# Epiphany-f/PSL-SLAM

Hardware: AMD Instinct MI355X
Metric: frames/sec ORB+line extract+match, 640x480 RGB-D, 1/2/4/8 MI355X (higher is better)
Workload: dtype u8; 1 GPU; configs[2]: 640x480 synthetic structure scene at the configured line load ('sticks': non-overlapping high-contrast bars), ORB 1000/1.2/8 FAST 20/7 + LSD (LSD_REFINE_ADV) / merge / top-200 / LBD + LIL pairing + RGB-D line glue (isLineGood, crossings, planes) extract, SearchByProjection(cur,last) + LSDmatcher::match, frames resident in HBM; scene=sticks, distinct_frames_per_batch=256, streams=1, launcher=none, multi_gpu=single GPU, lsd_refine=LSD_REFINE_ADV, lbd_sample_bytes_per_frame=2654242

## Files before the change

### psl-slam_amd/csrc/pslfe_line.hip

```cpp
#include <math.h>
#include <stdlib.h>
#include <string.h>

#include <algorithm>
#include <mutex>
#include <vector>

#include "line_kernels2.h"
#include "line_kernels3.h"
#include "pslfe_internal.h"

#ifndef PSL_NFA_COUNT_WGS
#define PSL_NFA_COUNT_WGS 4
#endif
#define PSL_GROW_LDS_USED_MAX (144u * 1024u)
#ifndef PSL_GROW_HELPER_FRAMES
#define PSL_GROW_HELPER_FRAMES 64
#endif

#define PSL_GROW_LDS_DEVICES 64
static std::mutex g_grow_lds_mu;
static size_t g_grow_lds_attr[PSL_GROW_LDS_DEVICES];

static hipError_t psl_grow_lds_allow(int device, size_t bytes) {
    if (bytes <= 64u * 1024u) return hipSuccess;
    if (device < 0 || device >= PSL_GROW_LDS_DEVICES) return hipErrorInvalidDevice;
    std::lock_guard<std::mutex> lock(g_grow_lds_mu);
    if (bytes <= g_grow_lds_attr[device]) return hipSuccess;
    const hipError_t e = hipFuncSetAttribute(reinterpret_cast<const void*>(&k_lsd_grow4<3, 1>), hipFuncAttributeMaxDynamicSharedMemorySize, (int)bytes);
    if (e == hipSuccess) g_grow_lds_attr[device] = bytes;
    return e;
}

struct pslfe_line {
    pslfe_ctx* ctx = nullptr;
    int numOctaves = 1, nfeatures = 200, max_batch = 1;
    float scale = 1.2f;
    double min_line_length = 0;
    int refine = 2;
    std::vector<float> scaleF, invScaleF, sigma2, invSigma2;

    int gw = 0, gh = 0;
    LineParams P;
    size_t in_fstride = 0;
    int in_pitch = 0;
    int last_nframes = 0;

    uint8_t* d_in = nullptr;
    double* d_scaled = nullptr;
    float* d_angdeg = nullptr;
    double* d_modgrad = nullptr;
    float2* d_trig = nullptr;
    float2* d_seedt = nullptr;
    uint8_t* d_used = nullptr;
    uint32_t* d_reg = nullptr;
    LsdnTables NT = {};
    double* d_lgamma = nullptr;
    double* d_sctab = nullptr;
    double* d_rects = nullptr;
    int* d_nrect = nullptr;
    int* d_weight = nullptr;
    int* d_order = nullptr;
    float* d_segtmp = nullptr;
    uint8_t* d_keep = nullptr;
    int2* d_counts = nullptr;
    int2* d_count0 = nullptr;
    uint16_t* d_ulist = nullptr;
    int* d_ucount = nullptr;
    double* d_vals = nullptr;
    double2* d_sstate = nullptr;
    LsdnSeries* d_slist = nullptr;
    LsdnSeries* d_stmp = nullptr;
    int* d_lcount = nullptr;
    float* d_seg = nullptr;
    int* d_nseg = nullptr;
    MergeScratch M = {};
    PslKeyLine* d_kls = nullptr;
    uint8_t* d_ldesc = nullptr;
    float* d_fdesc = nullptr;
    double* d_lineEq = nullptr;
    int* d_nkl = nullptr;
    int* d_status = nullptr;
    short2* d_dxy = nullptr;
    float* d_rawfans = nullptr;
    float* d_fans = nullptr;
    int* d_nfans = nullptr;
    float* d_tmplines = nullptr;

    PslDeviceBuffers mem;

    void release() {
        mem.release();
        gw = gh = 0;
        last_nframes = 0;
    }

    int prepare(int w, int h) {
        if (w == gw && h == gh) return PSLFE_OK;
        PSL_REQUIRE(w >= 16 && h >= 16 && w <= 8192 && h <= 8192, PSLFE_E_INVALID, "line: image %dx%d out of range", w, h);
        LineParams Q;
        memset(&Q, 0, sizeof(Q));
        Q.w = w; Q.h = h;
        Q.W = (int)nearbyint(w * 0.8);
        Q.H = (int)nearbyint(h * 0.8);
        Q.maxseg = PSL_MERGE_NMAX;
        Q.maxkl = std::max(1024, nfeatures);
        Q.nfeatures = nfeatures;
        {
            const double sigma = 0.6 / 0.8;
            const int ksize = 1 + 2 * (int)ceil(sigma * sqrt(2 * 3.0 * log(10.0)));
            PSL_REQUIRE(ksize == 7, PSLFE_E_INVALID, "line: unexpected LSD kernel size %d", ksize);
            const double scale2X = -0.5 / (sigma * sigma);
            double sum = 0;
            for (int i = 0; i < 7; ++i) { const double x = i - 3.0; Q.gk[i] = exp(scale2X * x * x); sum += Q.gk[i]; }
            sum = 1. / sum;
            for (int i = 0; i < 7; ++i) Q.gk[i] *= sum;
        }
        Q.prec = PSL_PI * 22.5 / 180;
        Q.p = 22.5 / 180;
        Q.rho = 2.0 / sin(Q.prec);
        {
            double q = Q.rho * Q.rho;
            while (sqrt(nextafter(q, INFINITY)) <= Q.rho) q = nextafter(q, INFINITY);
            while (sqrt(q) > Q.rho) q = nextafter(q, 0.0);
            Q.rho_q = q;
        }
        const double LOG_NT = 5 * (log10((double)Q.W) + log10((double)Q.H)) / 2 + log10(11.0);
        Q.min_reg_size = (int)(size_t)(-LOG_NT / log10(Q.p));
        Q.log_nt = LOG_NT;
        Q.refine = refine;
        {
            float cf[5];
            double sum = 0;
            for (int i = 0; i < 5; ++i) { const double x = i - 2.0; cf[i] = (float)exp(-0.5 * x * x); sum += cf[i]; }
            sum = 1. / sum;
            for (int i = 0; i < 5; ++i) { cf[i] = (float)(cf[i] * sum); Q.lbdK[i] = (int)nearbyint((double)cf[i] * 256.0); }
        }
        {
            const int wb = 7, nb = 9;
            double u = (wb * 3 - 1) / 2, sigma = (wb * 2 + 1) / 2, inv = -1 / (2 * sigma * sigma);
            for (int i = 0; i < wb * 3; ++i) { const double d = i - u; Q.gaussL[i] = (float)exp(d * d * inv); }
            u = (nb * wb - 1) / 2; sigma = u; inv = -1 / (2 * sigma * sigma);
            for (int i = 0; i < nb * wb; ++i) { const double d = i - u; Q.gaussG[i] = (float)exp(d * d * inv); }
        }
        PSL_HIP(hipSetDevice(ctx->device));
        PSL_HIP(hipStreamSynchronize(ctx->stream));
        release();
        if (int rc = allocate(Q, w, h)) { release(); return rc; }
        P = Q;
        gw = w; gh = h;
        last_nframes = 0;
        return PSLFE_OK;
    }

    int allocate(LineParams& Q, int w, int h) {
        const size_t F = (size_t)max_batch, npx = (size_t)Q.W * Q.H, N = PSL_MERGE_NMAX;
        in_pitch = (int)psl_align_up(w, 16);
        in_fstride = psl_align_up((size_t)in_pitch * h, 256);
        static const double sctab[444] = {
#include "psl_sincostab.inc"
        };
        const int lgn = 1 << 16;
        std::vector<double> lg((size_t)lgn, 0.0);
        for (int i = 1; i < lgn; ++i) lg[i] = lsdn_log_gamma((double)i);
        lg.resize((size_t)lgn + 3 * PSL_NFA_NP + PSL_RATIO_BMAX);
        for (int i = 1; i < PSL_RATIO_BMAX; ++i) lg[(size_t)lgn + 3 * PSL_NFA_NP + i] = 1.0 / (double)i;
        double pj = Q.p;
        for (int j = 0; j < PSL_NFA_NP; ++j, pj = pj / 2) {
            lg[(size_t)lgn + j] = psl_log(pj); lg[(size_t)lgn + PSL_NFA_NP + j] = psl_log(1.0 - pj); lg[(size_t)lgn + 2 * PSL_NFA_NP + j] = psl_log10(pj);
        }
        mem.alloc(d_in, in_fstride * F, "d_in");
        mem.alloc(d_scaled, npx * std::min<size_t>(F, PSL_LSD_SUBBATCH), "d_scaled");
        mem.alloc(d_angdeg, npx * F, "d_angdeg");
        mem.alloc(d_modgrad, npx * F, "d_modgrad");
        mem.alloc(d_trig, npx * F, "d_trig");
        mem.alloc(d_seedt, npx * F, "d_seedt");
        mem.alloc(d_used, npx * F, "d_used");
        mem.alloc(d_reg, npx * F, "d_reg");
        mem.alloc(d_seg, (size_t)Q.maxseg * 4 * F, "d_seg");
        mem.alloc(d_nseg, F, "d_nseg");
        mem.alloc(d_rects, (size_t)Q.maxseg * PSL_LSD_RECT_F64 * F, "d_rects");
        mem.alloc(d_nrect, F, "d_nrect");
        mem.alloc(d_weight, F, "d_weight");
        mem.alloc(d_order, F, "d_order");
        mem.alloc(d_segtmp, (size_t)Q.maxseg * 4 * F, "d_segtmp");
        mem.alloc(d_keep, (size_t)Q.maxseg * F, "d_keep");
        mem.alloc(d_counts, (size_t)Q.maxseg * 5 * F, "d_counts");
        mem.alloc(d_count0, (size_t)Q.maxseg * F, "d_count0");
        mem.alloc(d_ulist, (size_t)Q.maxseg * 2 * F, "d_ulist");
        mem.alloc(d_ucount, 5 * F, "d_ucount");
        mem.alloc(d_vals, (size_t)Q.maxseg * 5 * F, "d_vals");
        mem.alloc(d_sstate, (size_t)Q.maxseg * 5 * F, "d_sstate");
        mem.alloc(d_slist, (size_t)Q.maxseg * 5 * F, "d_slist");
        mem.alloc(d_stmp, (size_t)Q.maxseg * 5 * F, "d_stmp");
        mem.alloc(d_lcount, F * (PSL_NFA_NCLS + 1), "d_lcount");
        mem.alloc(d_sctab, sizeof(sctab) / sizeof(double), "d_sctab");
        mem.alloc(d_lgamma, lg.size(), "d_lgamma");
        mem.alloc(M.lines0, F * N * 4, "M.lines0");
        mem.alloc(M.lines1, F * N * 4, "M.lines1");
        mem.alloc(M.merged, F * N * 4, "M.merged");
        mem.alloc(M.angles, F * N, "M.angles");
        mem.alloc(M.length, F * N, "M.length");
        mem.alloc(M.order, F * N, "M.order");
        mem.alloc(M.pos, F * N, "M.pos");
        mem.alloc(M.adj, F * N * (N / 32), "M.adj");
        mem.alloc(M.code, F * N, "M.code");
        mem.alloc(M.clist, F * PSL_MERGE_CLMAX, "M.clist");
        mem.alloc(M.coff, F * (2 * N + 2), "M.coff");
        mem.alloc(M.work, F * 4 * N, "M.work");
        mem.alloc(M.bits, F * (N / 32), "M.bits");
        mem.alloc(M.stage, F * N, "M.stage");
        mem.alloc(d_kls, F * Q.maxkl, "d_kls");
        mem.alloc(d_ldesc, F * Q.maxkl * 32, "d_ldesc");
        mem.alloc(d_fdesc, F * Q.maxkl * 72, "d_fdesc");
        mem.alloc(d_lineEq, F * Q.maxkl * 3, "d_lineEq");
        mem.alloc(d_nkl, F, "d_nkl");
        mem.alloc(d_status, F, "d_status");
        mem.alloc(d_dxy, F * (size_t)w * h, "d_dxy");
        mem.alloc(d_rawfans, F * PSL_FAN_CAP * 4, "d_rawfans");
        mem.alloc(d_fans, F * PSL_FAN_CAP * 4, "d_fans");
        mem.alloc(d_nfans, F, "d_nfans");
        mem.alloc(d_tmplines, N * 4, "d_tmplines");
        if (int rc = mem.check("line")) return rc;
        PSL_HIP(hipMemcpy(d_sctab, sctab, sizeof(sctab), hipMemcpyHostToDevice));
        Q.sctab = d_sctab;
        PSL_HIP(hipMemcpy(d_lgamma, lg.data(), lg.size() * sizeof(double), hipMemcpyHostToDevice));
        NT.lg = d_lgamma; NT.logs = d_lgamma + lgn; NT.lg_n = lgn; NT.p0 = Q.p; NT.log_nt = Q.log_nt; NT.inv = d_lgamma + lgn + 3 * PSL_NFA_NP;
        return PSLFE_OK;
    }

    int run_lsd(const uint8_t* d_gray, int nframes, int w, int h, int stride, size_t frame_stride) {
        int rc = prepare(w, h);
        if (rc) return rc;
        PSL_HIP(hipSetDevice(ctx->device));
        hipStream_t st = ctx->stream;
        const unsigned F = (unsigned)nframes;
        {
            PSL_HIP(hipMemsetAsync(d_used, 0, (size_t)P.W * P.H * F, st));
            P.singles = F <= PSL_GROW_HELPER_FRAMES;
            P.full_grad = nframes == 1;
            const bool ordered = F > PSL_GROW_HELPER_FRAMES;
            if (ordered) PSL_HIP(hipMemsetAsync(d_weight, 0, (size_t)F * sizeof(int), st));
            const unsigned tx = (P.W + 63) / 64, ty = (P.H + 15) / 16, gy = (P.H + PSL_GRAD_TH - 1) / PSL_GRAD_TH;
            const size_t npx = (size_t)P.W * P.H;
            for (unsigned f0 = 0; f0 < F; f0 += PSL_LSD_SUBBATCH) {
                const unsigned n = std::min<unsigned>(PSL_LSD_SUBBATCH, F - f0);
                const int xcd = n >= 8 ? 1 : 0;
                const size_t po = (size_t)f0 * npx;
                {
                    PSL_STAGE_BEGIN(ctx, "line.lsd_scale");
                    k_lsd_scale_tiled<<<xcd ? dim3(8, tx * ty, (n + 7) / 8) : dim3(tx, ty, n), 256, 0, st>>>(P, d_gray + (size_t)f0 * frame_stride, stride, frame_stride,
                                                                                                             d_scaled, (int)n, xcd);
                    PSL_STAGE_END(ctx, "line.lsd_scale");
                }
                {
                    PSL_STAGE_BEGIN(ctx, "line.lsd_grad");
                    k_lsd_grad<<<xcd ? dim3(8, tx * gy, (n + 7) / 8) : dim3(tx, gy, n), 256, 0, st>>>(P, d_scaled, d_angdeg + po, d_modgrad + po, d_trig + po, d_seedt + po,
                                                                                                      d_used + po, ordered ? d_weight + f0 : nullptr, (int)n, xcd);
                    PSL_STAGE_END(ctx, "line.lsd_grad");
                }
            }
            if (ordered) k_frame_order<<<1, 1024, 0, st>>>(d_weight, (int)F, P.W * P.H, d_order);
        }
        P.refine = refine;
        {
            PSL_STAGE_BEGIN(ctx, "line.lsd_grow");
            if (F <= PSL_GROW_HELPER_FRAMES) {
                const size_t ubytes = (((size_t)P.W * P.H + 31) >> 5) * 4;
                if (ubytes <= PSL_GROW_LDS_USED_MAX) {
                    PSL_HIP(psl_grow_lds_allow(ctx->device, ubytes));
                    k_lsd_grow4<3, 1><<<F, 256, ubytes, st>>>(P, d_angdeg, d_modgrad, d_trig, d_used, d_seedt, d_reg, d_seg, refine >= 2 ? d_nrect : d_nseg, d_rects, (int)F, nullptr);
                } else {
                    k_lsd_grow4<3, 0><<<F, 256, 0, st>>>(P, d_angdeg, d_modgrad, d_trig, d_used, d_seedt, d_reg, d_seg, refine >= 2 ? d_nrect : d_nseg, d_rects, (int)F, nullptr);
                }
            } else
                k_lsd_grow4<0, 0><<<F, 64, 0, st>>>(P, d_angdeg, d_modgrad, d_trig, d_used, d_seedt, d_reg, d_seg, refine >= 2 ? d_nrect : d_nseg, d_rects, (int)F,
                                                 d_order);
            PSL_STAGE_END(ctx, "line.lsd_grow");
            PSL_HIP(hipGetLastError());
        }
        if (refine >= 2) {
            const dim3 gc(F >= 64 ? PSL_NFA_COUNT_WGS : 128, F), gs(F >= 64 ? 1 : 4, F);
            PSL_HIP(hipMemsetAsync(d_ucount, 0, (size_t)5 * F * sizeof(int), st));
            auto ul = [&](int k) { return k >= 0 ? d_ulist + (size_t)(k & 1) * P.maxseg * F : nullptr; };
            auto uc = [&](int k) { return k >= 0 && k < 5 ? d_ucount + (size_t)k * F : nullptr; };
#define PSL_NFA_COUNT(PH)                                                                                                \
    {                                                                                                                    \
        PSL_STAGE_BEGIN(ctx, "line.nfa_count");                                                                          \
        k_lsd_nfa_count<PH><<<gc, 256, 0, st>>>(P, d_angdeg, d_rects, d_nrect, ul(PH + 1), uc(PH + 1), d_counts, d_count0); \
        PSL_STAGE_END(ctx, "line.nfa_count");                                                                            \
    }
#define PSL_NFA_EVAL(PH)                                                                                                 \
    {                                                                                                                    \
        PSL_STAGE_BEGIN(ctx, "line.nfa_eval");                                                                           \
        k_lsd_nfa_setup<PH><<<F, 256, 0, st>>>(P, NT, d_rects, d_nrect, ul(PH + 1), uc(PH + 1), d_counts, d_count0, d_vals, d_sstate, d_stmp, d_slist, d_lcount); \
        k_lsd_nfa_series<PH><<<dim3(PSL_NFA_NCLS, (F + PSL_NFA_FG - 1) / PSL_NFA_FG), 256, 0, st>>>(P, NT, (int)F, d_slist, d_lcount, d_sstate); \
        k_lsd_nfa_select<PH><<<gs, 256, 0, st>>>(P, NT.log_nt, d_rects, d_nrect, ul(PH + 1), uc(PH + 1), d_keep, d_vals, d_sstate, d_segtmp, \
                                                 PH < 3 ? ul(PH + 2) : nullptr, uc(PH + 2));                             \
        PSL_STAGE_END(ctx, "line.nfa_eval");                                                                             \
    }
            PSL_NFA_COUNT(PSL_NFA_FIRST)
            PSL_NFA_EVAL(PSL_NFA_FIRST)
            PSL_NFA_EVAL(-1)
            PSL_NFA_COUNT(0)
            PSL_NFA_EVAL(0)
            PSL_NFA_COUNT(1)
            PSL_NFA_EVAL(1)
            PSL_NFA_COUNT(2)
            PSL_NFA_EVAL(2)
            PSL_NFA_COUNT(3)
            PSL_NFA_EVAL(3)
#undef PSL_NFA_COUNT
#undef PSL_NFA_EVAL
            k_lsd_emit<<<F, 256, 0, st>>>(P, d_nrect, d_segtmp, d_keep, d_seg, d_nseg);
        }
        PSL_HIP(hipGetLastError());
        last_nframes = nframes;
        return PSLFE_OK;
    }

    int run_merge(int nframes) {
        PSL_HIP(hipSetDevice(ctx->device));
        PSL_STAGE_BEGIN(ctx, "line.merge");
        k_line_merge<PSL_MERGE_LDSN_SMALL><<<nframes, 256, 0, ctx->stream>>>(P, M, d_seg, d_nseg, d_kls, d_lineEq, d_nkl, d_status);
        k_line_merge<PSL_MERGE_LDSN><<<nframes, 256, 0, ctx->stream>>>(P, M, d_seg, d_nseg, d_kls, d_lineEq, d_nkl, d_status);
        PSL_STAGE_END(ctx, "line.merge");
        PSL_HIP(hipGetLastError());
        return PSLFE_OK;
    }

    int run_lbd(const uint8_t* d_gray, int nframes, int stride, size_t frame_stride, bool want_float) {
        PSL_HIP(hipSetDevice(ctx->device));
        hipStream_t st = ctx->stream;
        {
            PSL_STAGE_BEGIN(ctx, "line.lbd_pre");
            const unsigned tx = (P.w + 63) / 64, ty = (P.h + 31) / 32;
            const int xcd = nframes >= 8 ? 1 : 0;
            k_lbd_pre<<<xcd ? dim3(8, tx * ty, (nframes + 7) / 8) : dim3(tx, ty, nframes), 256, 0, st>>>(P, d_gray, stride, frame_stride, d_dxy, nframes, xcd);
            PSL_STAGE_END(ctx, "line.lbd_pre");
        }
        {
            PSL_STAGE_BEGIN(ctx, "line.lbd");
            const int per_frame = std::min(P.maxkl, std::max(P.nfeatures, 1));
            k_lbd<<<dim3((per_frame + 3) / 4, nframes), 256, 0, st>>>(P, d_dxy, d_kls, d_nkl, d_ldesc, want_float ? d_fdesc : nullptr);
            PSL_STAGE_END(ctx, "line.lbd");
        }
        PSL_HIP(hipGetLastError());
        return PSLFE_OK;
    }

    int run_pair(int nframes, float radius, float fanThr) {
        PSL_HIP(hipSetDevice(ctx->device));
        PSL_STAGE_BEGIN(ctx, "line.pair");
        k_lil_pair<<<nframes, 256, 0, ctx->stream>>>(reinterpret_cast<const float*>(d_kls) + 7, (size_t)P.maxkl * 17, 17, d_nkl, 0, radius, fanThr,
                                                     P.w, P.h, d_rawfans, d_fans, PSL_FAN_CAP, d_nfans);
        PSL_STAGE_END(ctx, "line.pair");
        PSL_HIP(hipGetLastError());
        return PSLFE_OK;
    }

    int upload(const uint8_t* gray, int nframes, int w, int h, int stride, size_t frame_stride) {
        int rc = prepare(w, h);
        if (rc) return rc;
        PSL_HIP(hipSetDevice(ctx->device));
        for (int f = 0; f < nframes; ++f)
            PSL_HIP(hipMemcpy2DAsync(d_in + (size_t)f * in_fstride, in_pitch, gray + (size_t)f * frame_stride, stride, w, h,
                                     hipMemcpyHostToDevice, ctx->stream));
        return PSLFE_OK;
    }
};

extern "C" {

int pslfe_line_create(pslfe_ctx* ctx, int numOctaves, float scale, int nLSDFeature, double min_line_length, int max_batch,
                      pslfe_line** out) {
    PSL_REQUIRE(ctx && out, PSLFE_E_INVALID, "pslfe_line_create: NULL argument");
    *out = nullptr;
    PSL_REQUIRE(numOctaves >= 1 && numOctaves <= PSLFE_MAX_LEVELS && nLSDFeature >= 1 && nLSDFeature <= 2048 && max_batch >= 1 && max_batch <= 65535,
                PSLFE_E_INVALID, "pslfe_line_create: numOctaves %d nLSDFeature %d max_batch %d", numOctaves, nLSDFeature, max_batch);
    PSL_REQUIRE(numOctaves == 1, PSLFE_E_INVALID,
                "pslfe_line_create: numOctaves %d: the reference's LSDDetector::detect(image, kls, (int)1.2f, numOctaves) throws for numOctaves > 1 "
                "(pyrDown to the source's own size); only numOctaves == 1 yields lines", numOctaves);
    pslfe_line* l = new pslfe_line();
    l->ctx = ctx; l->numOctaves = numOctaves; l->scale = scale; l->nfeatures = nLSDFeature; l->min_line_length = min_line_length;
    l->max_batch = max_batch;
    l->scaleF.resize(numOctaves); l->sigma2.resize(numOctaves); l->invScaleF.resize(numOctaves); l->invSigma2.resize(numOctaves);
    l->scaleF[0] = 1.0f; l->sigma2[0] = 1.0f;
    for (int i = 1; i < numOctaves; ++i) { l->scaleF[i] = l->scaleF[i - 1] * scale; l->sigma2[i] = l->scaleF[i] * l->scaleF[i]; }
    for (int i = 0; i < numOctaves; ++i) { l->invScaleF[i] = 1.0f / l->scaleF[i]; l->invSigma2[i] = 1.0f / l->sigma2[i]; }
    *out = l;
    return PSLFE_OK;
}

void pslfe_line_destroy(pslfe_line* line) {
    if (!line) return;
    (void)hipSetDevice(line->ctx->device);
    (void)hipStreamSynchronize(line->ctx->stream);
    delete line;
}

int pslfe_line_set_refine(pslfe_line* line, int refine) {
    PSL_REQUIRE(line, PSLFE_E_INVALID, "pslfe_line_set_refine: line is NULL");
    PSL_REQUIRE(refine == PSLFE_LSD_REFINE_STD || refine == PSLFE_LSD_REFINE_ADV, PSLFE_E_INVALID, "pslfe_line_set_refine: mode %d", refine);
    line->refine = refine;
    return PSLFE_OK;
}

int pslfe_line_levels(const pslfe_line* line) { return line ? line->numOctaves : PSLFE_E_INVALID; }
float pslfe_line_scale_factor(const pslfe_line* line) { return line ? line->scale : 0.f; }
int pslfe_line_scale_factors(const pslfe_line* line, float* scale, float* inv_scale, float* sigma2, float* inv_sigma2) {
    PSL_REQUIRE(line, PSLFE_E_INVALID, "pslfe_line_scale_factors: line is NULL");
    for (int i = 0; i < line->numOctaves; ++i) {
        if (scale) scale[i] = line->scaleF[i];
        if (inv_scale) inv_scale[i] = line->invScaleF[i];
        if (sigma2) sigma2[i] = line->sigma2[i];
        if (inv_sigma2) inv_sigma2[i] = line->invSigma2[i];
    }
    return PSLFE_OK;
}

int pslfe_lsd_detect(pslfe_line* line, const uint8_t* gray, int w, int h, int stride, float* segments, int cap, int* n) {
    PSL_REQUIRE(line && n, PSLFE_E_INVALID, "pslfe_lsd_detect: NULL argument");
    *n = 0;
    if (!gray || w <= 0 || h <= 0) return PSLFE_OK;
    PSL_REQUIRE(stride >= w, PSLFE_E_INVALID, "pslfe_lsd_detect: stride %d < width %d", stride, w);
    int rc = line->upload(gray, 1, w, h, stride, (size_t)stride * h);
    if (rc) return rc;
    rc = line->run_lsd(line->d_in, 1, w, h, line->in_pitch, line->in_fstride);
    if (rc) return rc;
    hipStream_t st = line->ctx->stream;
    int cnt = 0;
    PSL_HIP(hipMemcpyAsync(&cnt, line->d_nseg, sizeof(int), hipMemcpyDeviceToHost, st));
    PSL_HIP(hipStreamSynchronize(st));
    *n = cnt;
    PSL_REQUIRE(cnt <= cap, PSLFE_E_CAPACITY, "pslfe_lsd_detect: %d segments, capacity %d", cnt, cap);
    if (cnt > 0 && segments) {
        PSL_HIP(hipMemcpyAsync(segments, line->d_seg, (size_t)cnt * 4 * sizeof(float), hipMemcpyDeviceToHost, st));
        PSL_HIP(hipStreamSynchronize(st));
    }
    return PSLFE_OK;
}

int pslfe_line_debug_gradient(pslfe_line* line, int frame, int* W, int* H, double* scaled, float* angle_deg, double* modgrad) {
    PSL_REQUIRE(line && W && H, PSLFE_E_INVALID, "pslfe_line_debug_gradient: NULL argument");
    PSL_REQUIRE(line->last_nframes > 0 && frame >= 0 && frame < line->last_nframes, PSLFE_E_STATE, "pslfe_line_debug_gradient: frame %d", frame);
    PSL_HIP(hipSetDevice(line->ctx->device));
    PSL_HIP(hipStreamSynchronize(line->ctx->stream));
    *W = line->P.W; *H = line->P.H;
    const size_t npx = (size_t)line->P.W * line->P.H;
    if (scaled) {
        PSL_REQUIRE(line->last_nframes <= PSL_LSD_SUBBATCH, PSLFE_E_STATE, "pslfe_line_debug_gradient: the scaled image is kept for launches of at most %d frames", PSL_LSD_SUBBATCH);
        PSL_HIP(hipMemcpy(scaled, line->d_scaled + frame * npx, npx * sizeof(double), hipMemcpyDeviceToHost));
    }
    if (angle_deg) PSL_HIP(hipMemcpy(angle_deg, line->d_angdeg + frame * npx, npx * sizeof(float), hipMemcpyDeviceToHost));
    if (modgrad) PSL_HIP(hipMemcpy(modgrad, line->d_modgrad + frame * npx, npx * sizeof(double), hipMemcpyDeviceToHost));
    return PSLFE_OK;
}


int pslfe_line_debug_nfa(pslfe_line* line, int w, int h, int phase, int nframes, const int32_t* nrect, int rect_cap, const double* p_lognfa,
                         const int32_t* nk, double* vals, double* tail, double* log_nt) {
    PSL_REQUIRE(line && nrect && p_lognfa && nk && vals && tail, PSLFE_E_INVALID, "pslfe_line_debug_nfa: NULL argument");
    PSL_REQUIRE(phase == PSL_NFA_FIRST || (phase >= -1 && phase <= 3), PSLFE_E_INVALID, "pslfe_line_debug_nfa: phase %d", phase);
    PSL_REQUIRE(nframes >= 1 && nframes <= line->max_batch, PSLFE_E_INVALID, "pslfe_line_debug_nfa: nframes %d (max_batch %d)", nframes, line->max_batch);
    PSL_REQUIRE(rect_cap >= 1 && rect_cap <= PSL_MERGE_NMAX, PSLFE_E_INVALID, "pslfe_line_debug_nfa: rect_cap %d (at most %d)", rect_cap, PSL_MERGE_NMAX);
    const int TR = phase == PSL_NFA_FIRST ? 1 : 5;
    for (int f = 0; f < nframes; ++f) {
        PSL_REQUIRE(nrect[f] >= 0 && nrect[f] <= rect_cap, PSLFE_E_INVALID, "pslfe_line_debug_nfa: frame %d has %d rectangles (rect_cap %d)", f, nrect[f], rect_cap);
        for (int r = 0; r < nrect[f]; ++r) {
            const double p = p_lognfa[((size_t)f * rect_cap + r) * 2];
            PSL_REQUIRE(p > 0.0 && p < 1.0, PSLFE_E_INVALID, "pslfe_line_debug_nfa: frame %d rectangle %d: p %g", f, r, p);
            for (int t = 0; t < TR; ++t) {
                const int32_t* c = nk + (((size_t)f * rect_cap + r) * 5 + t) * 2;
                PSL_REQUIRE(c[0] < 0 || (c[1] >= 0 && c[1] <= c[0] && c[0] <= (1 << 24)), PSLFE_E_INVALID,
                            "pslfe_line_debug_nfa: frame %d rectangle %d trial %d: (n, k) = (%d, %d)", f, r, t, c[0], c[1]);
            }
        }
    }
    int rc = line->prepare(w, h);
    if (rc) return rc;
    PSL_HIP(hipSetDevice(line->ctx->device));
    hipStream_t st = line->ctx->stream;
    const LineParams& P = line->P;
    const size_t F = (size_t)nframes, N = (size_t)P.maxseg;
    std::vector<double> rects(F * N * PSL_LSD_RECT_F64, 0.0);
    std::vector<int2> cnt(F * N * TR, make_int2(-1, 0));
    std::vector<uint16_t> ulist(F * N, 0);
    for (size_t f = 0; f < F; ++f)
        for (int r = 0; r < nrect[f]; ++r) {
            const size_t o = f * N + r, s = f * rect_cap + r;
            rects[o * PSL_LSD_RECT_F64 + 9] = p_lognfa[s * 2];
            rects[o * PSL_LSD_RECT_F64 + 10] = p_lognfa[s * 2 + 1];
            for (int t = 0; t < TR; ++t) cnt[o * TR + t] = make_int2(nk[(s * 5 + t) * 2], nk[(s * 5 + t) * 2 + 1]);
            ulist[f * N + r] = (uint16_t)(nrect[f] - 1 - r);
        }
    PSL_HIP(hipMemcpyAsync(line->d_rects, rects.data(), rects.size() * sizeof(double), hipMemcpyHostToDevice, st));
    PSL_HIP(hipMemcpyAsync(line->d_nrect, nrect, F * sizeof(int), hipMemcpyHostToDevice, st));
    PSL_HIP(hipMemcpyAsync(phase == PSL_NFA_FIRST ? line->d_count0 : line->d_counts, cnt.data(), cnt.size() * sizeof(int2), hipMemcpyHostToDevice, st));
    uint16_t* d_ul = nullptr;
    int* d_uc = nullptr;
    if (phase != PSL_NFA_FIRST) {
        d_ul = line->d_ulist + (size_t)((phase + 1) & 1) * N * F;
        d_uc = line->d_ucount + (size_t)(phase + 1) * F;
        PSL_HIP(hipMemcpyAsync(d_ul, ulist.data(), ulist.size() * sizeof(uint16_t), hipMemcpyHostToDevice, st));
        PSL_HIP(hipMemcpyAsync(d_uc, nrect, F * sizeof(int), hipMemcpyHostToDevice, st));
    }
#define PSL_NFA_DEBUG_EVAL(PH)                                                                                                                  \
    case PH:                                                                                                                                    \
        k_lsd_nfa_setup<PH><<<F, 256, 0, st>>>(P, line->NT, line->d_rects, line->d_nrect, d_ul, d_uc, line->d_counts, line->d_count0, line->d_vals, \
                                               line->d_sstate, line->d_stmp, line->d_slist, line->d_lcount);                                    \
        k_lsd_nfa_series<PH><<<dim3(PSL_NFA_NCLS, (F + PSL_NFA_FG - 1) / PSL_NFA_FG), 256, 0, st>>>(P, line->NT, (int)F, line->d_slist, line->d_lcount, \
                                                                                                    line->d_sstate);                            \
        break;
    switch (phase) {
        PSL_NFA_DEBUG_EVAL(PSL_NFA_FIRST)
        PSL_NFA_DEBUG_EVAL(-1)
        PSL_NFA_DEBUG_EVAL(0)
        PSL_NFA_DEBUG_EVAL(1)
        PSL_NFA_DEBUG_EVAL(2)
        PSL_NFA_DEBUG_EVAL(3)
    }
#undef PSL_NFA_DEBUG_EVAL
    PSL_HIP(hipGetLastError());
    std::vector<double> v(F * N * 5);
    std::vector<double2> ss(F * N * 5);
    PSL_HIP(hipMemcpyAsync(v.data(), line->d_vals, v.size() * sizeof(double), hipMemcpyDeviceToHost, st));
    PSL_HIP(hipMemcpyAsync(ss.data(), line->d_sstate, ss.size() * sizeof(double2), hipMemcpyDeviceToHost, st));
    PSL_HIP(hipStreamSynchronize(st));
    for (size_t f = 0; f < F; ++f)
        for (int r = 0; r < nrect[f]; ++r)
            for (int t = 0; t < TR; ++t) {
                vals[((size_t)f * rect_cap + r) * 5 + t] = v[(f * N + r) * 5 + t];
                tail[((size_t)f * rect_cap + r) * 5 + t] = ss[(f * N + r) * 5 + t].x;
            }
    if (log_nt) *log_nt = line->NT.log_nt;
    return PSLFE_OK;
}

int pslfe_line_extract_batch_device(pslfe_line* line, const uint8_t* d_gray, int nframes, int w, int h, int stride, size_t frame_stride) {
    PSL_REQUIRE(line && d_gray, PSLFE_E_INVALID, "pslfe_line_extract_batch_device: NULL argument");
    PSL_REQUIRE(nframes >= 1 && nframes <= line->max_batch, PSLFE_E_INVALID, "pslfe_line_extract_batch_device: nframes %d (max_batch %d)", nframes, line->max_batch);
    PSL_REQUIRE(stride >= w && (nframes == 1 || frame_stride >= (size_t)stride * h), PSLFE_E_INVALID, "pslfe_line_extract_batch_device: strides");
    int rc = line->run_lsd(d_gray, nframes, w, h, stride, frame_stride);
    if (rc) return rc;
    if ((rc = line->run_merge(nframes))) return rc;
    return line->run_lbd(d_gray, nframes, stride, frame_stride, false);
}

int pslfe_line_results_device(pslfe_line* line, const PslKeyLine** d_kls, const uint8_t** d_desc, const double** d_lineEq,
                              const int32_t** d_counts, int* kl_cap) {
    PSL_REQUIRE(line, PSLFE_E_INVALID, "pslfe_line_results_device: line is NULL");
    PSL_REQUIRE(line->last_nframes > 0, PSLFE_E_STATE, "pslfe_line_results_device: no batch extracted yet");
    if (d_kls) *d_kls = line->d_kls;
    if (d_desc) *d_desc = line->d_ldesc;
    if (d_lineEq) *d_lineEq = line->d_lineEq;
    if (d_counts) *d_counts = line->d_nkl;
    if (kl_cap) *kl_cap = line->P.maxkl;
    return PSLFE_OK;
}

int pslfe_line_fetch(pslfe_line* line, int frame, PslKeyLine* kls, uint8_t* desc, double* lineEq, int cap, int* n, int* status) {
    PSL_REQUIRE(line && n, PSLFE_E_INVALID, "pslfe_line_fetch: NULL argument");
    PSL_REQUIRE(line->last_nframes > 0 && frame >= 0 && frame < line->last_nframes, PSLFE_E_STATE, "pslfe_line_fetch: frame %d", frame);
    PSL_HIP(hipSetDevice(line->ctx->device));
    hipStream_t st = line->ctx->stream;
    int cnt = 0, stt = 0;
    PSL_HIP(hipMemcpyAsync(&cnt, line->d_nkl + frame, sizeof(int), hipMemcpyDeviceToHost, st));
    PSL_HIP(hipMemcpyAsync(&stt, line->d_status + frame, sizeof(int), hipMemcpyDeviceToHost, st));
    PSL_HIP(hipStreamSynchronize(st));
    *n = cnt;
    if (status) *status = stt;
    PSL_REQUIRE(cnt <= cap, PSLFE_E_CAPACITY, "pslfe_line_fetch: %d keylines, capacity %d", cnt, cap);
    if (cnt > 0) {
        const size_t o = (size_t)frame * line->P.maxkl;
        if (kls) PSL_HIP(hipMemcpyAsync(kls, line->d_kls + o, (size_t)cnt * sizeof(PslKeyLine), hipMemcpyDeviceToHost, st));
        if (desc) PSL_HIP(hipMemcpyAsync(desc, line->d_ldesc + o * 32, (size_t)cnt * 32, hipMemcpyDeviceToHost, st));
        if (lineEq) PSL_HIP(hipMemcpyAsync(lineEq, line->d_lineEq + o * 3, (size_t)cnt * 3 * sizeof(double), hipMemcpyDeviceToHost, st));
        PSL_HIP(hipStreamSynchronize(st));
    }
    return PSLFE_OK;
}

int pslfe_line_segments_fetch(pslfe_line* line, int frame, float* segments, int cap, int* n) {
    PSL_REQUIRE(line && n, PSLFE_E_INVALID, "pslfe_line_segments_fetch: NULL argument");
    PSL_REQUIRE(line->last_nframes > 0 && frame >= 0 && frame < line->last_nframes, PSLFE_E_STATE, "pslfe_line_segments_fetch: frame %d", frame);
    PSL_HIP(hipSetDevice(line->ctx->device));
    hipStream_t st = line->ctx->stream;
    int cnt = 0;
    PSL_HIP(hipMemcpyAsync(&cnt, line->d_nseg + frame, sizeof(int), hipMemcpyDeviceToHost, st));
    PSL_HIP(hipStreamSynchronize(st));
    *n = cnt;
    PSL_REQUIRE(cnt <= cap && cnt <= line->P.maxseg, PSLFE_E_CAPACITY, "pslfe_line_segments_fetch: %d segments, capacity %d (list %d)", cnt, cap,
                line->P.maxseg);
    if (cnt > 0 && segments) {
        PSL_HIP(hipMemcpyAsync(segments, line->d_seg + (size_t)frame * line->P.maxseg * 4, (size_t)cnt * 4 * sizeof(float), hipMemcpyDeviceToHost, st));
        PSL_HIP(hipStreamSynchronize(st));
    }
    return PSLFE_OK;
}

int pslfe_line_extract(pslfe_line* line, const uint8_t* gray, int w, int h, int stride, PslKeyLine* kls, uint8_t* desc, double* lineEq,
                       int cap, int* n) {
    PSL_REQUIRE(line && n, PSLFE_E_INVALID, "pslfe_line_extract: NULL argument");
    *n = 0;
    if (!gray || w <= 0 || h <= 0) return PSLFE_OK;
    PSL_REQUIRE(stride >= w, PSLFE_E_INVALID, "pslfe_line_extract: stride %d < width %d", stride, w);
    int rc = line->upload(gray, 1, w, h, stride, (size_t)stride * h);
    if (rc) return rc;
    rc = pslfe_line_extract_batch_device(line, line->d_in, 1, w, h, line->in_pitch, line->in_fstride);
    if (rc) return rc;
    return pslfe_line_fetch(line, 0, kls, desc, lineEq, cap, n, nullptr);
}

int pslfe_line_optimize_and_merge(pslfe_line* line, const float* segments, int nseg, int w, int h, PslKeyLine* kls, int cap, int* n) {
    PSL_REQUIRE(line && n && (nseg == 0 || segments), PSLFE_E_INVALID, "pslfe_line_optimize_and_merge: NULL argument");
    *n = 0;
    PSL_REQUIRE(nseg >= 0 && nseg <= PSL_MERGE_NMAX, PSLFE_E_CAPACITY, "pslfe_line_optimize_and_merge: %d segments (max %d)", nseg, PSL_MERGE_NMAX);
    int rc = line->prepare(w, h);
    if (rc) return rc;
    PSL_HIP(hipSetDevice(line->ctx->device));
    hipStream_t st = line->ctx->stream;
    if (nseg) PSL_HIP(hipMemcpyAsync(line->d_seg, segments, (size_t)nseg * 4 * sizeof(float), hipMemcpyHostToDevice, st));
    PSL_HIP(hipMemcpyAsync(line->d_nseg, &nseg, sizeof(int), hipMemcpyHostToDevice, st));
    PSL_HIP(hipStreamSynchronize(st));
    const int keep = line->P.nfeatures;
    line->P.nfeatures = line->P.maxkl;
    rc = line->run_merge(1);
    line->P.nfeatures = keep;
    if (rc) return rc;
    line->last_nframes = 1;
    return pslfe_line_fetch(line, 0, kls, nullptr, nullptr, cap, n, nullptr);
}

int pslfe_lbd_compute(pslfe_line* line, const uint8_t* gray, int w, int h, int stride, const PslKeyLine* kls, int nkl, uint8_t* desc,
                      float* fdesc) {
    PSL_REQUIRE(line && gray && (nkl == 0 || (kls && desc)), PSLFE_E_INVALID, "pslfe_lbd_compute: NULL argument");
    if (nkl == 0) return PSLFE_OK;
    PSL_REQUIRE(stride >= w, PSLFE_E_INVALID, "pslfe_lbd_compute: stride %d < width %d", stride, w);
    int rc = line->upload(gray, 1, w, h, stride, (size_t)stride * h);
    if (rc) return rc;
    PSL_REQUIRE(nkl <= line->P.maxkl, PSLFE_E_CAPACITY, "pslfe_lbd_compute: %d keylines (max %d)", nkl, line->P.maxkl);
    hipStream_t st = line->ctx->stream;
    PSL_HIP(hipMemcpyAsync(line->d_kls, kls, (size_t)nkl * sizeof(PslKeyLine), hipMemcpyHostToDevice, st));
    PSL_HIP(hipMemcpyAsync(line->d_nkl, &nkl, sizeof(int), hipMemcpyHostToDevice, st));
    PSL_HIP(hipStreamSynchronize(st));
    const int keep = line->P.nfeatures;
    line->P.nfeatures = std::max(keep, nkl);
    rc = line->run_lbd(line->d_in, 1, line->in_pitch, line->in_fstride, fdesc != nullptr);
    line->P.nfeatures = keep;
    if (rc) return rc;
    PSL_HIP(hipMemcpyAsync(desc, line->d_ldesc, (size_t)nkl * 32, hipMemcpyDeviceToHost, st));
    if (fdesc) PSL_HIP(hipMemcpyAsync(fdesc, line->d_fdesc, (size_t)nkl * 72 * sizeof(float), hipMemcpyDeviceToHost, st));
    PSL_HIP(hipStreamSynchronize(st));
    line->last_nframes = 1;
    return PSLFE_OK;
}

int pslfe_line_debug_sobel(pslfe_line* line, int frame, int16_t* dx, int16_t* dy) {
    PSL_REQUIRE(line && dx && dy, PSLFE_E_INVALID, "pslfe_line_debug_sobel: NULL argument");
    PSL_REQUIRE(line->last_nframes > 0 && frame >= 0 && frame < line->last_nframes, PSLFE_E_STATE, "pslfe_line_debug_sobel: frame %d", frame);
    PSL_HIP(hipSetDevice(line->ctx->device));
    PSL_HIP(hipStreamSynchronize(line->ctx->stream));
    const size_t npx = (size_t)line->P.w * line->P.h;
    std::vector<short2> tmp(npx);
    PSL_HIP(hipMemcpy(tmp.data(), line->d_dxy + frame * npx, npx * sizeof(short2), hipMemcpyDeviceToHost));
    for (size_t i = 0; i < npx; ++i) { dx[i] = tmp[i].x; dy[i] = tmp[i].y; }
    return PSLFE_OK;
}

int pslfe_lil_pair(pslfe_line* line, const float* lines, int nlines, float radius, float fanThr, int imgCols, int imgRows, float* fans,
                   int cap, int* nfans) {
    PSL_REQUIRE(line && nfans && (nlines == 0 || lines), PSLFE_E_INVALID, "pslfe_lil_pair: NULL argument");
    *nfans = 0;
    if (nlines == 0) return PSLFE_OK;
    PSL_REQUIRE(nlines <= PSL_MERGE_NMAX, PSLFE_E_CAPACITY, "pslfe_lil_pair: %d lines (max %d)", nlines, PSL_MERGE_NMAX);
    int rc = line->prepare(line->gw > 0 ? line->gw : std::max(imgCols, 16), line->gh > 0 ? line->gh : std::max(imgRows, 16));
    if (rc) return rc;
    PSL_HIP(hipSetDevice(line->ctx->device));
    hipStream_t st = line->ctx->stream;
    PSL_HIP(hipMemcpyAsync(line->d_tmplines, lines, (size_t)nlines * 4 * sizeof(float), hipMemcpyHostToDevice, st));
    PSL_HIP(hipStreamSynchronize(st));
    {
        PSL_STAGE_BEGIN(line->ctx, "line.pair");
        k_lil_pair<<<1, 256, 0, st>>>(line->d_tmplines, 0, 4, nullptr, nlines, radius, fanThr, imgCols, imgRows, line->d_rawfans, line->d_fans,
                                      PSL_FAN_CAP, line->d_nfans);
        PSL_STAGE_END(line->ctx, "line.pair");
    }
    PSL_HIP(hipGetLastError());
    int k = 0;
    PSL_HIP(hipMemcpyAsync(&k, line->d_nfans, sizeof(int), hipMemcpyDeviceToHost, st));
    PSL_HIP(hipStreamSynchronize(st));
    *nfans = k;
    PSL_REQUIRE(k <= cap, PSLFE_E_CAPACITY, "pslfe_lil_pair: %d fans, capacity %d", k, cap);
    if (k > 0 && fans) {
        PSL_HIP(hipMemcpyAsync(fans, line->d_fans, (size_t)k * 4 * sizeof(float), hipMemcpyDeviceToHost, st));
        PSL_HIP(hipStreamSynchronize(st));
    }
    return PSLFE_OK;
}

int pslfe_line_pair_batch_device(pslfe_line* line, float radius, float fanThr) {
    PSL_REQUIRE(line, PSLFE_E_INVALID, "pslfe_line_pair_batch_device: line is NULL");
    PSL_REQUIRE(line->last_nframes > 0, PSLFE_E_STATE, "pslfe_line_pair_batch_device: no batch extracted yet");
    return line->run_pair(line->last_nframes, radius, fanThr);
}

int pslfe_line_fans_device(pslfe_line* line, const float** d_fans, const int32_t** d_nfans, int* fan_stride) {
    PSL_REQUIRE(line, PSLFE_E_INVALID, "pslfe_line_fans_device: line is NULL");
    PSL_REQUIRE(line->last_nframes > 0, PSLFE_E_STATE, "pslfe_line_fans_device: no batch extracted yet");
    if (d_fans) *d_fans = line->d_fans;
    if (d_nfans) *d_nfans = line->d_nfans;
    if (fan_stride) *fan_stride = PSL_FAN_CAP;
    return PSLFE_OK;
}

int pslfe_line_fans_fetch(pslfe_line* line, int frame, float* fans, int cap, int* nfans) {
    PSL_REQUIRE(line && nfans, PSLFE_E_INVALID, "pslfe_line_fans_fetch: NULL argument");
    PSL_REQUIRE(line->last_nframes > 0 && frame >= 0 && frame < line->last_nframes, PSLFE_E_STATE, "pslfe_line_fans_fetch: frame %d", frame);
    PSL_HIP(hipSetDevice(line->ctx->device));
    hipStream_t st = line->ctx->stream;
    int k = 0;
    PSL_HIP(hipMemcpyAsync(&k, line->d_nfans + frame, sizeof(int), hipMemcpyDeviceToHost, st));
    PSL_HIP(hipStreamSynchronize(st));
    *nfans = k;
    PSL_REQUIRE(k <= cap, PSLFE_E_CAPACITY, "pslfe_line_fans_fetch: %d fans, capacity %d", k, cap);
    if (k > 0 && fans) {
        PSL_HIP(hipMemcpyAsync(fans, line->d_fans + (size_t)frame * PSL_FAN_CAP * 4, (size_t)k * 4 * sizeof(float), hipMemcpyDeviceToHost, st));
        PSL_HIP(hipStreamSynchronize(st));
    }
    return PSLFE_OK;
}


int pslfe_line_match_batch_device(pslfe_line* line, int shift, float nnr, int32_t* d_matches12, int32_t* d_nmatches) {
    PSL_REQUIRE(line && d_matches12 && d_nmatches, PSLFE_E_INVALID, "pslfe_line_match_batch_device: NULL argument");
    PSL_REQUIRE(line->last_nframes > 0, PSLFE_E_STATE, "pslfe_line_match_batch_device: no batch extracted yet");
    PSL_HIP(hipSetDevice(line->ctx->device));
    hipStream_t st = line->ctx->stream;
    const int F = line->last_nframes, cap = line->P.maxkl;
    PSL_HIP(hipMemsetAsync(d_nmatches, 0, (size_t)F * sizeof(int), st));
    {
        PSL_STAGE_BEGIN(line->ctx, "line.match");
        const int qmax = std::min(cap, line->P.nfeatures);
        k_line_match_batch<<<dim3(F, (qmax + 3) / 4), 256, 0, st>>>(line->d_ldesc, line->d_nkl, cap, F, shift, nnr, d_matches12, d_nmatches);
        PSL_STAGE_END(line->ctx, "line.match");
    }
    PSL_HIP(hipGetLastError());
    return PSLFE_OK;
}

}
```

Measured before the change: 33020 frames/s.

## Split line detect/merge/LBD into two frame pieces on concurrent streams

```diff
diff --git a/psl-slam_amd/csrc/pslfe_line.hip b/psl-slam_amd/csrc/pslfe_line.hip
--- a/psl-slam_amd/csrc/pslfe_line.hip
+++ b/psl-slam_amd/csrc/pslfe_line.hip
@@ -17,6 +17,7 @@
 #ifndef PSL_GROW_HELPER_FRAMES
 #define PSL_GROW_HELPER_FRAMES 64
 #endif
+constexpr unsigned PSL_LINE_PIECES = 2;
 
 #define PSL_GROW_LDS_DEVICES 64
 static std::mutex g_grow_lds_mu;
@@ -229,75 +230,115 @@
         return PSLFE_OK;
     }
 
-    int run_lsd(const uint8_t* d_gray, int nframes, int w, int h, int stride, size_t frame_stride) {
+    struct Part {
+        unsigned f0, n, F;
+        hipStream_t st;
+        float* angdeg; double* modgrad; float2* trig; float2* seedt; uint8_t* used; uint32_t* reg;
+        double* rects; int* nrect; int* weight; int* order;
+        int2* counts; int2* count0; uint16_t* ulist; int* ucount; double* vals; double2* sstate; LsdnSeries* slist; LsdnSeries* stmp; int* lcount;
+        uint8_t* keep; float* segtmp; float* seg; int* nseg;
+        MergeScratch M;
+        PslKeyLine* kls; uint8_t* ldesc; float* fdesc; double* lineEq; int* nkl; int* status; short2* dxy;
+        size_t maxseg;
+        uint16_t* ul(int k) const { return k >= 0 ? ulist + (size_t)(k & 1) * maxseg * F : nullptr; }
+        int* uc(int k) const { return k >= 0 && k < 5 ? ucount + (size_t)k * F : nullptr; }
+    };
+
+    Part part(unsigned f0, unsigned n, unsigned F, hipStream_t st) const {
+        const size_t npx = (size_t)P.W * P.H, S = (size_t)P.maxseg, K = (size_t)P.maxkl, N = PSL_MERGE_NMAX;
+        auto at = [f0](auto* base, size_t per_frame) { return base + (size_t)f0 * per_frame; };
+        Part p;
+        p.f0 = f0; p.n = n; p.F = F; p.st = st; p.maxseg = S;
+        p.angdeg = at(d_angdeg, npx); p.modgrad = at(d_modgrad, npx); p.trig = at(d_trig, npx); p.seedt = at(d_seedt, npx);
+        p.used = at(d_used, npx); p.reg = at(d_reg, npx);
+        p.rects = at(d_rects, S * PSL_LSD_RECT_F64); p.nrect = at(d_nrect, 1); p.weight = at(d_weight, 1); p.order = at(d_order, 1);
+        p.counts = at(d_counts, S * 5); p.count0 = at(d_count0, S); p.ulist = at(d_ulist, S); p.ucount = at(d_ucount, 1);
+        p.vals = at(d_vals, S * 5); p.sstate = at(d_sstate, S * 5); p.slist = at(d_slist, S * 5); p.stmp = at(d_stmp, S * 5);
+        p.lcount = at(d_lcount, PSL_NFA_NCLS + 1);
+        p.keep = at(d_keep, S); p.segtmp = at(d_segtmp, S * 4); p.seg = at(d_seg, S * 4); p.nseg = at(d_nseg, 1);
+        p.M.lines0 = at(M.lines0, N * 4); p.M.lines1 = at(M.lines1, N * 4); p.M.merged = at(M.merged, N * 4);
+        p.M.angles = at(M.angles, N); p.M.length = at(M.length, N); p.M.order = at(M.order, N); p.M.pos = at(M.pos, N);
+        p.M.adj = at(M.adj, N * (N / 32)); p.M.code = at(M.code, N); p.M.clist = at(M.clist, PSL_MERGE_CLMAX);
+        p.M.coff = at(M.coff, 2 * N + 2); p.M.work = at(M.work, 4 * N); p.M.bits = at(M.bits, N / 32); p.M.stage = at(M.stage, N);
+        p.kls = at(d_kls, K); p.ldesc = at(d_ldesc, K * 32); p.fdesc = at(d_fdesc, K * 72); p.lineEq = at(d_lineEq, K * 3);
+        p.nkl = at(d_nkl, 1); p.status = at(d_status, 1); p.dxy = at(d_dxy, (size_t)P.w * P.h);
+        return p;
+    }
+    Part whole(int nframes) const { return part(0, (unsigned)nframes, (unsigned)nframes, ctx->stream); }
+
+    int run_grad(const uint8_t* d_gray, int nframes, int w, int h, int stride, size_t frame_stride) {
         int rc = prepare(w, h);
         if (rc) return rc;
         PSL_HIP(hipSetDevice(ctx->device));
         hipStream_t st = ctx->stream;
         const unsigned F = (unsigned)nframes;
+        PSL_HIP(hipMemsetAsync(d_used, 0, (size_t)P.W * P.H * F, st));
+        P.singles = F <= PSL_GROW_HELPER_FRAMES;
+        P.full_grad = nframes == 1;
+        P.refine = refine;
+        const bool ordered = F > PSL_GROW_HELPER_FRAMES;
+        if (ordered) PSL_HIP(hipMemsetAsync(d_weight, 0, (size_t)F * sizeof(int), st));
+        if (refine >= 2) PSL_HIP(hipMemsetAsync(d_ucount, 0, (size_t)5 * F * sizeof(int), st));
+        const unsigned tx = (P.W + 63) / 64, ty = (P.H + 15) / 16, gy = (P.H + PSL_GRAD_TH - 1) / PSL_GRAD_TH;
+        const size_t npx = (size_t)P.W * P.H;
+        for (unsigned f0 = 0; f0 < F; f0 += PSL_LSD_SUBBATCH) {
+            const unsigned n = std::min<unsigned>(PSL_LSD_SUBBATCH, F - f0);
+            const int xcd = n >= 8 ? 1 : 0;
+            const size_t po = (size_t)f0 * npx;
+            {
+                PSL_STAGE_BEGIN(ctx, "line.lsd_scale");
+                k_lsd_scale_tiled<<<xcd ? dim3(8, tx * ty, (n + 7) / 8) : dim3(tx, ty, n), 256, 0, st>>>(P, d_gray + (size_t)f0 * frame_stride, stride, frame_stride,
+                                                                                                         d_scaled, (int)n, xcd);
+                PSL_STAGE_END(ctx, "line.lsd_scale");
+            }
+            {
+                PSL_STAGE_BEGIN(ctx, "line.lsd_grad");
+                k_lsd_grad<<<xcd ? dim3(8, tx * gy, (n + 7) / 8) : dim3(tx, gy, n), 256, 0, st>>>(P, d_scaled, d_angdeg + po, d_modgrad + po, d_trig + po, d_seedt + po,
+                                                                                                  d_used + po, ordered ? d_weight + f0 : nullptr, (int)n, xcd);
+                PSL_STAGE_END(ctx, "line.lsd_grad");
+            }
+        }
+        PSL_HIP(hipGetLastError());
+        return PSLFE_OK;
+    }
+
+    int run_detect(const Part& p) {
+        hipStream_t st = p.st;
+        const unsigned n = p.n;
+        int* const ngrow = refine >= 2 ? p.nrect : p.nseg;
+        const bool ordered = n > PSL_GROW_HELPER_FRAMES;
+        if (ordered) k_frame_order<<<1, 1024, 0, st>>>(p.weight, (int)n, P.W * P.H, p.order);
         {
-            PSL_HIP(hipMemsetAsync(d_used, 0, (size_t)P.W * P.H * F, st));
-            P.singles = F <= PSL_GROW_HELPER_FRAMES;
-            P.full_grad = nframes == 1;
-            const bool ordered = F > PSL_GROW_HELPER_FRAMES;
-            if (ordered) PSL_HIP(hipMemsetAsync(d_weight, 0, (size_t)F * sizeof(int), st));
-            const unsigned tx = (P.W + 63) / 64, ty = (P.H + 15) / 16, gy = (P.H + PSL_GRAD_TH - 1) / PSL_GRAD_TH;
-            const size_t npx = (size_t)P.W * P.H;
-            for (unsigned f0 = 0; f0 < F; f0 += PSL_LSD_SUBBATCH) {
-                const unsigned n = std::min<unsigned>(PSL_LSD_SUBBATCH, F - f0);
-                const int xcd = n >= 8 ? 1 : 0;
-                const size_t po = (size_t)f0 * npx;
-                {
-                    PSL_STAGE_BEGIN(ctx, "line.lsd_scale");
-                    k_lsd_scale_tiled<<<xcd ? dim3(8, tx * ty, (n + 7) / 8) : dim3(tx, ty, n), 256, 0, st>>>(P, d_gray + (size_t)f0 * frame_stride, stride, frame_stride,
-                                                                                                             d_scaled, (int)n, xcd);
-                    PSL_STAGE_END(ctx, "line.lsd_scale");
-                }
-                {
-                    PSL_STAGE_BEGIN(ctx, "line.lsd_grad");
-                    k_lsd_grad<<<xcd ? dim3(8, tx * gy, (n + 7) / 8) : dim3(tx, gy, n), 256, 0, st>>>(P, d_scaled, d_angdeg + po, d_modgrad + po, d_trig + po, d_seedt + po,
-                                                                                                      d_used + po, ordered ? d_weight + f0 : nullptr, (int)n, xcd);
-                    PSL_STAGE_END(ctx, "line.lsd_grad");
-                }
-            }
-            if (ordered) k_frame_order<<<1, 1024, 0, st>>>(d_weight, (int)F, P.W * P.H, d_order);
-        }
-        P.refine = refine;
-        {
-            PSL_STAGE_BEGIN(ctx, "line.lsd_grow");
-            if (F <= PSL_GROW_HELPER_FRAMES) {
+            PSL_STAGE_BEGIN_ON(ctx, "line.lsd_grow", st);
+            if (!ordered) {
                 const size_t ubytes = (((size_t)P.W * P.H + 31) >> 5) * 4;
                 if (ubytes <= PSL_GROW_LDS_USED_MAX) {
                     PSL_HIP(psl_grow_lds_allow(ctx->device, ubytes));
-                    k_lsd_grow4<3, 1><<<F, 256, ubytes, st>>>(P, d_angdeg, d_modgrad, d_trig, d_used, d_seedt, d_reg, d_seg, refine >= 2 ? d_nrect : d_nseg, d_rects, (int)F, nullptr);
+                    k_lsd_grow4<3, 1><<<n, 256, ubytes, st>>>(P, p.angdeg, p.modgrad, p.trig, p.used, p.seedt, p.reg, p.seg, ngrow, p.rects, (int)n, nullptr);
                 } else {
-                    k_lsd_grow4<3, 0><<<F, 256, 0, st>>>(P, d_angdeg, d_modgrad, d_trig, d_used, d_seedt, d_reg, d_seg, refine >= 2 ? d_nrect : d_nseg, d_rects, (int)F, nullptr);
+                    k_lsd_grow4<3, 0><<<n, 256, 0, st>>>(P, p.angdeg, p.modgrad, p.trig, p.used, p.seedt, p.reg, p.seg, ngrow, p.rects, (int)n, nullptr);
                 }
             } else
-                k_lsd_grow4<0, 0><<<F, 64, 0, st>>>(P, d_angdeg, d_modgrad, d_trig, d_used, d_seedt, d_reg, d_seg, refine >= 2 ? d_nrect : d_nseg, d_rects, (int)F,
-                                                 d_order);
-            PSL_STAGE_END(ctx, "line.lsd_grow");
+                k_lsd_grow4<0, 0><<<n, 64, 0, st>>>(P, p.angdeg, p.modgrad, p.trig, p.used, p.seedt, p.reg, p.seg, ngrow, p.rects, (int)n, p.order);
+            PSL_STAGE_END_ON(ctx, "line.lsd_grow", st);
             PSL_HIP(hipGetLastError());
         }
         if (refine >= 2) {
-            const dim3 gc(F >= 64 ? PSL_NFA_COUNT_WGS : 128, F), gs(F >= 64 ? 1 : 4, F);
-            PSL_HIP(hipMemsetAsync(d_ucount, 0, (size_t)5 * F * sizeof(int), st));
-            auto ul = [&](int k) { return k >= 0 ? d_ulist + (size_t)(k & 1) * P.maxseg * F : nullptr; };
-            auto uc = [&](int k) { return k >= 0 && k < 5 ? d_ucount + (size_t)k * F : nullptr; };
+            const dim3 gc(n >= 64 ? PSL_NFA_COUNT_WGS : 128, n), gs(n >= 64 ? 1 : 4, n);
 #define PSL_NFA_COUNT(PH)                                                                                                \
     {                                                                                                                    \
-        PSL_STAGE_BEGIN(ctx, "line.nfa_count");                                                                          \
-        k_lsd_nfa_count<PH><<<gc, 256, 0, st>>>(P, d_angdeg, d_rects, d_nrect, ul(PH + 1), uc(PH + 1), d_counts, d_count0); \
-        PSL_STAGE_END(ctx, "line.nfa_count");                                                                            \
+        PSL_STAGE_BEGIN_ON(ctx, "line.nfa_count", st);                                                                   \
+        k_lsd_nfa_count<PH><<<gc, 256, 0, st>>>(P, p.angdeg, p.rects, p.nrect, p.ul(PH + 1), p.uc(PH + 1), p.counts, p.count0); \
+        PSL_STAGE_END_ON(ctx, "line.nfa_count", st);                                                                     \
     }
 #define PSL_NFA_EVAL(PH)                                                                                                 \
     {                                                                                                                    \
-        PSL_STAGE_BEGIN(ctx, "line.nfa_eval");                                                                           \
-        k_lsd_nfa_setup<PH><<<F, 256, 0, st>>>(P, NT, d_rects, d_nrect, ul(PH + 1), uc(PH + 1), d_counts, d_count0, d_vals, d_sstate, d_stmp, d_slist, d_lcount); \
-        k_lsd_nfa_series<PH><<<dim3(PSL_NFA_NCLS, (F + PSL_NFA_FG - 1) / PSL_NFA_FG), 256, 0, st>>>(P, NT, (int)F, d_slist, d_lcount, d_sstate); \
-        k_lsd_nfa_select<PH><<<gs, 256, 0, st>>>(P, NT.log_nt, d_rects, d_nrect, ul(PH + 1), uc(PH + 1), d_keep, d_vals, d_sstate, d_segtmp, \
-                                                 PH < 3 ? ul(PH + 2) : nullptr, uc(PH + 2));                             \
-        PSL_STAGE_END(ctx, "line.nfa_eval");                                                                             \
+        PSL_STAGE_BEGIN_ON(ctx, "line.nfa_eval", st);                                                                    \
+        k_lsd_nfa_setup<PH><<<n, 256, 0, st>>>(P, NT, p.rects, p.nrect, p.ul(PH + 1), p.uc(PH + 1), p.counts, p.count0, p.vals, p.sstate, p.stmp, p.slist, p.lcount); \
+        k_lsd_nfa_series<PH><<<dim3(PSL_NFA_NCLS, (n + PSL_NFA_FG - 1) / PSL_NFA_FG), 256, 0, st>>>(P, NT, (int)n, p.slist, p.lcount, p.sstate); \
+        k_lsd_nfa_select<PH><<<gs, 256, 0, st>>>(P, NT.log_nt, p.rects, p.nrect, p.ul(PH + 1), p.uc(PH + 1), p.keep, p.vals, p.sstate, p.segtmp, \
+                                                 PH < 3 ? p.ul(PH + 2) : nullptr, p.uc(PH + 2));                         \
+        PSL_STAGE_END_ON(ctx, "line.nfa_eval", st);                                                                      \
     }
             PSL_NFA_COUNT(PSL_NFA_FIRST)
             PSL_NFA_EVAL(PSL_NFA_FIRST)
@@ -312,40 +353,79 @@
             PSL_NFA_EVAL(3)
 #undef PSL_NFA_COUNT
 #undef PSL_NFA_EVAL
-            k_lsd_emit<<<F, 256, 0, st>>>(P, d_nrect, d_segtmp, d_keep, d_seg, d_nseg);
+            k_lsd_emit<<<n, 256, 0, st>>>(P, p.nrect, p.segtmp, p.keep, p.seg, p.nseg);
         }
         PSL_HIP(hipGetLastError());
+        return PSLFE_OK;
+    }
+
+    int run_lsd(const uint8_t* d_gray, int nframes, int w, int h, int stride, size_t frame_stride) {
+        int rc = run_grad(d_gray, nframes, w, h, stride, frame_stride);
+        if (rc) return rc;
+        if ((rc = run_detect(whole(nframes)))) return rc;
         last_nframes = nframes;
         return PSLFE_OK;
     }
 
-    int run_merge(int nframes) {
+    int run_merge(const Part& p) {
         PSL_HIP(hipSetDevice(ctx->device));
-        PSL_STAGE_BEGIN(ctx, "line.merge");
-        k_line_merge<PSL_MERGE_LDSN_SMALL><<<nframes, 256, 0, ctx->stream>>>(P, M, d_seg, d_nseg, d_kls, d_lineEq, d_nkl, d_status);
-        k_line_merge<PSL_MERGE_LDSN><<<nframes, 256, 0, ctx->stream>>>(P, M, d_seg, d_nseg, d_kls, d_lineEq, d_nkl, d_status);
-        PSL_STAGE_END(ctx, "line.merge");
+        PSL_STAGE_BEGIN_ON(ctx, "line.merge", p.st);
+        k_line_merge<PSL_MERGE_LDSN_SMALL><<<p.n, 256, 0, p.st>>>(P, p.M, p.seg, p.nseg, p.kls, p.lineEq, p.nkl, p.status);
+        k_line_merge<PSL_MERGE_LDSN><<<p.n, 256, 0, p.st>>>(P, p.M, p.seg, p.nseg, p.kls, p.lineEq, p.nkl, p.status);
+        PSL_STAGE_END_ON(ctx, "line.merge", p.st);
         PSL_HIP(hipGetLastError());
         return PSLFE_OK;
     }
 
-    int run_lbd(const uint8_t* d_gray, int nframes, int stride, size_t frame_stride, bool want_float) {
+    int run_lbd(const Part& p, const uint8_t* d_gray, int stride, size_t frame_stride, bool want_float) {
         PSL_HIP(hipSetDevice(ctx->device));
-        hipStream_t st = ctx->stream;
+        hipStream_t st = p.st;
+        const int n = (int)p.n;
         {
-            PSL_STAGE_BEGIN(ctx, "line.lbd_pre");
+            PSL_STAGE_BEGIN_ON(ctx, "line.lbd_pre", st);
             const unsigned tx = (P.w + 63) / 64, ty = (P.h + 31) / 32;
-            const int xcd = nframes >= 8 ? 1 : 0;
-            k_lbd_pre<<<xcd ? dim3(8, tx * ty, (nframes + 7) / 8) : dim3(tx, ty, nframes), 256, 0, st>>>(P, d_gray, stride, frame_stride, d_dxy, nframes, xcd);
-            PSL_STAGE_END(ctx, "line.lbd_pre");
+            const int xcd = n >= 8 ? 1 : 0;
+            k_lbd_pre<<<xcd ? dim3(8, tx * ty, (n + 7) / 8) : dim3(tx, ty, n), 256, 0, st>>>(P, d_gray + (size_t)p.f0 * frame_stride, stride, frame_stride, p.dxy, n, xcd);
+            PSL_STAGE_END_ON(ctx, "line.lbd_pre", st);
         }
         {
-            PSL_STAGE_BEGIN(ctx, "line.lbd");
+            PSL_STAGE_BEGIN_ON(ctx, "line.lbd", st);
             const int per_frame = std::min(P.maxkl, std::max(P.nfeatures, 1));
-            k_lbd<<<dim3((per_frame + 3) / 4, nframes), 256, 0, st>>>(P, d_dxy, d_kls, d_nkl, d_ldesc, want_float ? d_fdesc : nullptr);
-            PSL_STAGE_END(ctx, "line.lbd");
+            k_lbd<<<dim3((per_frame + 3) / 4, n), 256, 0, st>>>(P, p.dxy, p.kls, p.nkl, p.ldesc, want_float ? p.fdesc : nullptr);
+            PSL_STAGE_END_ON(ctx, "line.lbd", st);
         }
         PSL_HIP(hipGetLastError());
+        return PSLFE_OK;
+    }
+
+    int run_part(const Part& p, const uint8_t* d_gray, int stride, size_t frame_stride) {
+        int rc = run_detect(p);
+        if (rc) return rc;
+        if ((rc = run_merge(p))) return rc;
+        return run_lbd(p, d_gray, stride, frame_stride, false);
+    }
+
+    int run_extract(const uint8_t* d_gray, int nframes, int w, int h, int stride, size_t frame_stride) {
+        int rc = run_grad(d_gray, nframes, w, h, stride, frame_stride);
+        if (rc) return rc;
+        const unsigned F = (unsigned)nframes;
+        if (F < 2 * (PSL_GROW_HELPER_FRAMES + 1) || ctx->profile) {
+            if ((rc = run_part(whole(nframes), d_gray, stride, frame_stride))) return rc;
+        } else {
+            const unsigned pieces = std::min<unsigned>(PSL_LINE_PIECES, F / (PSL_GROW_HELPER_FRAMES + 1));
+            PSL_HIP(hipEventRecord(ctx->ev_fork, ctx->stream));
+            PSL_HIP(hipStreamWaitEvent(ctx->aux_stream, ctx->ev_fork, 0));
+            for (unsigned i = 0; i < pieces && !rc; ++i) {
+                const unsigned f0 = (unsigned)((size_t)F * i / pieces), f1 = (unsigned)((size_t)F * (i + 1) / pieces);
+                rc = run_part(part(f0, f1 - f0, F, i & 1 ? ctx->aux_stream : ctx->stream), d_gray, stride, frame_stride);
+            }
+            const hipError_t ej = hipEventRecord(ctx->ev_join, ctx->aux_stream);
+            const hipError_t ew = ej == hipSuccess ? hipStreamWaitEvent(ctx->stream, ctx->ev_join, 0) : ej;
+            if (ew != hipSuccess) (void)hipStreamSynchronize(ctx->aux_stream);
+            if (rc) return rc;
+            PSL_HIP(ew);
+        }
+        last_nframes = nframes;
         return PSLFE_OK;
     }
 
@@ -541,10 +621,7 @@
     PSL_REQUIRE(line && d_gray, PSLFE_E_INVALID, "pslfe_line_extract_batch_device: NULL argument");
     PSL_REQUIRE(nframes >= 1 && nframes <= line->max_batch, PSLFE_E_INVALID, "pslfe_line_extract_batch_device: nframes %d (max_batch %d)", nframes, line->max_batch);
     PSL_REQUIRE(stride >= w && (nframes == 1 || frame_stride >= (size_t)stride * h), PSLFE_E_INVALID, "pslfe_line_extract_batch_device: strides");
-    int rc = line->run_lsd(d_gray, nframes, w, h, stride, frame_stride);
-    if (rc) return rc;
-    if ((rc = line->run_merge(nframes))) return rc;
-    return line->run_lbd(d_gray, nframes, stride, frame_stride, false);
+    return line->run_extract(d_gray, nframes, w, h, stride, frame_stride);
 }
 
 int pslfe_line_results_device(pslfe_line* line, const PslKeyLine** d_kls, const uint8_t** d_desc, const double** d_lineEq,
@@ -625,7 +702,7 @@
     PSL_HIP(hipStreamSynchronize(st));
     const int keep = line->P.nfeatures;
     line->P.nfeatures = line->P.maxkl;
-    rc = line->run_merge(1);
+    rc = line->run_merge(line->whole(1));
     line->P.nfeatures = keep;
     if (rc) return rc;
     line->last_nframes = 1;
@@ -646,7 +723,7 @@
     PSL_HIP(hipStreamSynchronize(st));
     const int keep = line->P.nfeatures;
     line->P.nfeatures = std::max(keep, nkl);
-    rc = line->run_lbd(line->d_in, 1, line->in_pitch, line->in_fstride, fdesc != nullptr);
+    rc = line->run_lbd(line->whole(1), line->d_in, line->in_pitch, line->in_fstride, fdesc != nullptr);
     line->P.nfeatures = keep;
     if (rc) return rc;
     PSL_HIP(hipMemcpyAsync(desc, line->d_ldesc, (size_t)nkl * 32, hipMemcpyDeviceToHost, st));
```

After: 35030 frames/s, median of 6. 1.06x the previous value.
